# noahares/raxtax

Measured on AMD Instinct MI355X. Metric: classified queries/sec (whole node), higher is better.
Workload: dtype u32 bit-planes + f64

## Files before the change

### raxtax_amd/csrc/rtx_api_batch.hip

```cpp
#include "rtx_index.hpp"

#ifndef RTX_B2_HEAVY_PER_ATILE
#define RTX_B2_HEAVY_PER_ATILE 4u
#endif

namespace rtxi {

int bind(rtx_index *ix) {
    if (!ix) { set_error("null index handle"); return RTX_ERR_INVALID; }
    RTX_HIP(hipSetDevice(ix->device));
    return RTX_OK;
}

int ensure_events(rtx_index *ix, size_t count) {
    while (ix->events.size() < count) {
        hipEvent_t e;
        RTX_HIP(hipEventCreate(&e));
        ix->events.push_back(e);
    }
    return RTX_OK;
}


SubBatch sub_batch_of(rtx_index *ix, uint32_t sb, bool timed) {
// ... 524 lines not shown
        RTX_HIP(hipMemcpyAsync(&r.h_fin_sub[b.sb], r.d_fin_cursor.p, 8, hipMemcpyDeviceToHost, s));
    return RTX_OK;
}

static WalkParams walk_params(rtx_index *ix, const SubBatch &b, const double *prefix) {
    rtx_index::ResultSet &r = ix->res();
    WalkParams wp{};
    wp.status = r.d_status.p;
    wp.q0 = b.q0;
    wp.prefix = prefix;
    wp.n_bnd = ix->n_bnd;
    wp.rec = ix->d_noderec.p;
    wp.arena = r.d_arena.p;
    const bool side = b.cls->side;
    wp.arena_cap = side ? r.arena_cap : r.side_base;
    wp.arena_cursor = r.d_cursor.p + (side ? 1 : 0);
    wp.sub_alloc = !side && b.nq >= kWalkSubMinQueries && r.arena_cap < (1ull << 32) ? ix->d_sub_alloc.p : nullptr;
    wp.n_rows = r.d_n_rows.p;
    wp.row_start = r.d_row_start.p;
    wp.flags_out = r.d_flags.p;
    return wp;
}
static int reset_sub_alloc(rtx_index *ix, hipStream_t s) {
    if (ix->d_sub_alloc.p) RTX_HIP(hipMemsetAsync(ix->d_sub_alloc.p, 0, (size_t)kWalkSubAllocs * kWalkSubStride * 8, s));
    return RTX_OK;
}

int enqueue_walk(rtx_index *ix, const SubBatch &b, const double *prefix, hipStream_t s) {
    const WalkParams wp = walk_params(ix, b, prefix);
    int rc_r = wp.sub_alloc ? reset_sub_alloc(ix, s) : RTX_OK;
    if (rc_r) return rc_r;
    if (b.timed_all) RTX_HIP(hipEventRecord(stage_event(ix, b, RTX_STAGE_LINEAGE_WALK, 0), s));
    launch_lineage_walk(s, wp, b.nq);
    if (b.timed_all) RTX_HIP(hipEventRecord(stage_event(ix, b, RTX_STAGE_LINEAGE_WALK, 1), s));
    return RTX_OK;
}

int order_batch(rtx_index *ix, bool cluster) {
    const uint32_t n = (uint32_t)ix->n_q;
    rtx_index::ResultSet &r = ix->res();
    int rc;
    if ((rc = r.d_perm.alloc(n)) || (rc = r.d_iperm.alloc(n))) return rc;
    const bool multi = ix->n_cls > 1;
    const bool sketch = cluster && n > 2;
    if (sketch || multi) {
        if ((rc = ix->d_skey_in.alloc(n)) || (rc = ix->d_skey_out.alloc(n)) || (rc = ix->d_sidx.alloc(n))) return rc;
        size_t tmp = 0;
        if (cluster_sort(ix->stream, nullptr, &tmp, ix->d_skey_in.p, ix->d_skey_out.p, ix->d_sidx.p, r.d_perm.p, n, multi)) {
            set_error("radix sort: size query failed");
            return RTX_ERR_HIP;
        }
        if (ix->d_sort_tmp.n < tmp && (rc = ix->d_sort_tmp.alloc(tmp + 256))) return rc;
        if (sketch) {
            launch_sketch(ix->stream, ix->d_bases.p, ix->in[ix->cur_in].d_base_off.p, n, ix->d_skey_in.p, ix->d_sidx.p);
            if (ix->d_loc_table.p && ix->locator_opt)
                launch_locator(ix->stream, ix->d_bases.p, ix->in[ix->cur_in].d_base_off.p, n, ix->d_loc_table.p, ix->n_total, ix->d_skey_in.p);
        }
        if (multi) launch_class_keys(ix->stream, ix->d_skey_in.p, ix->in[ix->cur_in].d_base_off.p, n, ix->key_lim, !sketch, ix->d_sidx.p);
        tmp = ix->d_sort_tmp.n;
        if (cluster_sort(ix->stream, ix->d_sort_tmp.p, &tmp, ix->d_skey_in.p, ix->d_skey_out.p, ix->d_sidx.p, r.d_perm.p, n, multi)) {
            set_error("radix sort of the query sketches failed");
            return RTX_ERR_HIP;
        }
        launch_invert_perm(ix->stream, r.d_perm.p, n, r.d_iperm.p);
    } else {
        launch_identity_perm(ix->stream, n, r.d_perm.p, r.d_iperm.p);
    }
    RTX_HIP(hipGetLastError());
    return RTX_OK;
}

void record_batch(rtx_index *ix) {
    rtx_index::ResultSet &r = ix->res();
    r.n_q = ix->n_q;
    r.n_user = ix->strand_used ? ix->n_user : ix->n_q;
    r.has_peak = false;
    r.has_nearest = false;
    r.has_identity = false;
    r.profiled = false;
    r.n_sub = ix->n_sub_total();
    r.n_side = 0;
    for (uint32_t c = 0; c < ix->n_cls; c++)
        if (ix->cls[c].side) r.n_side += ix->cls[c].n_sub;
    r.in_set = ix->cur_in;
    r.dev_exact = ix->dev_exact_used;
    r.stream_dl = false;
}

int begin_run(rtx_index *ix, uint32_t *n_sub_out, bool *timed_out, bool cluster) {
    int rc_p = plan_sub_batches(ix);
    if (rc_p) return rc_p;
    const uint32_t n_sub = ix->n_sub_total();
    record_batch(ix);
    rtx_index::ResultSet &r = ix->res();
    const bool timed = n_sub <= 4096;
    if (timed) {
        int rc = ensure_events(ix, (size_t)n_sub * RTX_NUM_STAGES * 2);
        if (rc) return rc;
    }
    const bool ev_all = timed && ix->stage_timing;
    if (ev_all) RTX_HIP(hipEventRecord(ix->events[(size_t)RTX_STAGE_ORDER * 2], ix->stream));
    int rc_o = order_batch(ix, cluster);
    if (rc_o) return rc_o;
    if (ev_all) RTX_HIP(hipEventRecord(ix->events[(size_t)RTX_STAGE_ORDER * 2 + 1], ix->stream));
    {
        uint64_t n_side_q = 0;
        for (uint32_t c = 0; c < ix->n_cls; c++)
            if (ix->cls[c].side) n_side_q += ix->cls[c].n;
        const uint64_t side_rows = n_side_q ? n_side_q * kWalkMaxRows + 64 : 0;
// ... 696 lines not shown
```

### raxtax_amd/csrc/rtx_cluster.hip

```cpp
#include <cstring>

#include <hip/hip_runtime.h>
#include <rocprim/device/device_radix_sort.hpp>

#include "rtx_kernels.hpp"
#include "rtx_wave.hpp"

namespace rtx {

static constexpr int kSketchK = 12;
static constexpr uint32_t kSketchBits = 21;

__global__ __launch_bounds__(64) void sketch_kernel(const uint8_t *__restrict__ bases, const uint64_t *__restrict__ off,
                                                    uint64_t *__restrict__ keys, uint32_t *__restrict__ idx) {
    const uint32_t q = blockIdx.x, lane = threadIdx.x;
    const uint64_t b0 = off[q], len = off[q + 1] - b0;
    const uint8_t *seq = bases + b0;
    const uint32_t none = (1u << kSketchBits) - 1u;
    uint32_t m1 = none, m2 = none, m3 = none;
    if (len >= (uint64_t)kSketchK) {
        const uint64_t nwin = len - kSketchK + 1;
        const uint64_t wpl = (nwin + 63) / 64;
        const uint64_t w0 = (uint64_t)lane * wpl;
        const uint64_t w1 = w0 + wpl < nwin ? w0 + wpl : nwin;
        for (uint64_t i = w0; i < w1; i += 16) {
            unsigned long long v[4];
            __builtin_memcpy(v, seq + i, 32);
            const uint32_t nw = w1 - i < 16 ? (uint32_t)(w1 - i) : 16u;
            uint32_t code = 0, run = 0;
#pragma unroll
            for (int b = 0; b < 16 + kSketchK - 1; b++) {
                const uint32_t c = (uint32_t)(v[b >> 3] >> ((b & 7) * 8)) & 0xFFu;
                const bool ok = c == 1u || c == 2u || c == 4u || c == 8u;
                code = ((code << 2) | (((uint32_t)__ffs((int)c) - 1u) & 3u)) & 0xFFFFFFu;
                run = ok ? run + 1u : 0u;
                if (b >= kSketchK - 1 && (uint32_t)(b - (kSketchK - 1)) < nw && run >= (uint32_t)kSketchK) {
                    const uint64_t x = code;
                    const uint32_t h1 = (uint32_t)((x * 0x9E3779B97F4A7C15ull) >> (64 - kSketchBits));
                    const uint32_t h2 = (uint32_t)((x * 0xC2B2AE3D27D4EB4Full) >> (64 - kSketchBits));
                    const uint32_t h3 = (uint32_t)((x * 0x165667B19E3779F9ull) >> (64 - kSketchBits));
                    m1 = h1 < m1 ? h1 : m1;
                    m2 = h2 < m2 ? h2 : m2;
                    m3 = h3 < m3 ? h3 : m3;
                }
            }
        }
    }
#pragma unroll
    for (int d = 32; d >= 1; d >>= 1) {
        const uint32_t o1 = __shfl_xor(m1, d, 64), o2 = __shfl_xor(m2, d, 64), o3 = __shfl_xor(m3, d, 64);
        m1 = o1 < m1 ? o1 : m1;
        m2 = o2 < m2 ? o2 : m2;
        m3 = o3 < m3 ? o3 : m3;
    }
    if (lane == 0) {
        keys[q] = ((uint64_t)m1 << (2 * kSketchBits)) | ((uint64_t)m2 << kSketchBits) | m3;
        idx[q] = q;
    }
}

static constexpr uint32_t kLocNone = 0xFFFFFFFFu;
static constexpr uint32_t kLocMaxCount = 512;

__device__ __forceinline__ bool base_code(uint32_t c, uint32_t &two) {
    two = ((uint32_t)__ffs((int)c) - 1u) & 3u;
    return c == 1u || c == 2u || c == 4u || c == 8u;
}

__global__ __launch_bounds__(64) void loc_mark_kernel(const uint8_t *__restrict__ bases, const uint64_t *__restrict__ off,
                                                      uint64_t n_refs, uint32_t *__restrict__ pos_min, uint32_t *__restrict__ cnt) {
    const uint32_t lane = threadIdx.x;
    for (uint64_t r = blockIdx.x; r < n_refs; r += gridDim.x) {
        const uint64_t b0 = off[r], len = off[r + 1] - b0;
        if (len < (uint64_t)kSketchK) continue;
        const uint8_t *seq = bases + b0;
        const uint64_t nwin = len - kSketchK + 1;
        for (uint64_t w = lane; w < nwin; w += 64) {
            uint32_t code = 0;
            bool ok = true;
#pragma unroll
            for (int j = 0; j < kSketchK; j++) {
                uint32_t two;
                ok = base_code(seq[w + j], two) && ok;
                code = (code << 2) | two;
            }
            if (ok) {
                atomicMin(&pos_min[code], (uint32_t)r);
                atomicAdd(&cnt[code], 1u);
            }
        }
    }
}

__global__ __launch_bounds__(256) void loc_finish_kernel(uint32_t *__restrict__ pos_min, const uint32_t *__restrict__ cnt) {
    const uint32_t i = blockIdx.x * 256 + threadIdx.x;
    const uint32_t c = cnt[i];
    if (c == 0u || c > kLocMaxCount) pos_min[i] = kLocNone;
}

static constexpr uint32_t kLocMaxBins = 8192;
static constexpr uint32_t kLocFineDiv = 16;
static constexpr uint32_t kLocWin = 1024;
#ifndef RTX_LOC_STRIDE
#define RTX_LOC_STRIDE 2
#endif
static constexpr uint32_t kLocStride = RTX_LOC_STRIDE;

__device__ __forceinline__ void vote_bins(uint32_t *h, uint32_t b, bool valid, uint32_t lane) {
    unsigned long long pending = __ballot(valid);
#pragma unroll
    for (int r = 0; r < 2; r++) {
        if (!pending) return;
        const int first = __builtin_ctzll(pending);
        const uint32_t lead = (uint32_t)__builtin_amdgcn_readlane((int)b, first);
        const unsigned long long same = __ballot(valid && b == lead) & pending;
        if ((int)lane == first) atomicAdd(&h[lead >> 1], (uint32_t)__popcll(same) << ((lead & 1u) * 16u));
        pending &= ~same;
    }
    if ((pending >> lane) & 1ull) atomicAdd(&h[b >> 1], 1u << ((b & 1u) * 16u));
}

__global__ __launch_bounds__(64) void locator_kernel(const uint8_t *__restrict__ bases, const uint64_t *__restrict__ off,
                                                     const uint32_t *__restrict__ table, uint32_t bin_shift, uint32_t n_bins,
                                                     uint64_t *__restrict__ keys) {
    extern __shared__ __attribute__((aligned(16))) uint32_t h[];
    __shared__ uint32_t lcode[kLocWin / kLocStride];
    __shared__ uint32_t hf[kLocFineDiv + 2];
    const uint32_t q = blockIdx.x, lane = threadIdx.x;
    const uint64_t b0 = off[q], len = off[q + 1] - b0;
    if (len < (uint64_t)kSketchK) return;
    const uint64_t old_key = keys[q];
    const uint8_t *seq = bases + b0;
    const uint32_t nwin = (uint32_t)(len - kSketchK + 1 < (uint64_t)kLocWin ? len - kSketchK + 1 : kLocWin);
    const uint32_t words = n_bins / 2 + 2;
    for (uint32_t i = lane; i < (words + 3u) / 4u; i += 64) reinterpret_cast<uint4 *>(h)[i] = make_uint4(0u, 0u, 0u, 0u);
    if (lane < kLocFineDiv + 2) hf[lane] = 0;
    {
        const uint32_t wpl = (nwin + 63u) / 64u;
        const uint32_t w0 = lane * wpl, w1 = w0 + wpl < nwin ? w0 + wpl : nwin;
        static_assert(kLocWin <= 1024u && kLocWin % kLocStride == 0u, "a lane's run of windows fits one piece of 16");
        if (w0 < w1) {
            unsigned long long v[4];
            __builtin_memcpy(v, seq + w0, 32);
            const uint32_t nw = w1 - w0;
            uint32_t code = 0, run = 0;
#pragma unroll
            for (int b = 0; b < 16 + kSketchK - 1; b++) {
                uint32_t two;
                const bool ok = base_code((uint32_t)(v[b >> 3] >> ((b & 7) * 8)) & 0xFFu, two);
                code = ((code << 2) | two) & 0xFFFFFFu;
                run = ok ? run + 1u : 0u;
                if (b >= kSketchK - 1 && (uint32_t)(b - (kSketchK - 1)) < nw) {
                    const uint32_t w = w0 + (uint32_t)(b - (kSketchK - 1));
                    if (w % kLocStride == 0u) lcode[w / kLocStride] = run >= (uint32_t)kSketchK ? code : kLocNone;
                }
            }
        }
    }
    __builtin_amdgcn_fence(__ATOMIC_ACQ_REL, "wavefront");
    __builtin_amdgcn_wave_barrier();
    uint32_t any = 0;
    const uint32_t nlook = (nwin + kLocStride - 1u) / kLocStride;
    for (uint32_t j0 = 0; j0 < nlook; j0 += 256) {
        uint32_t pos[4];
#pragma unroll
        for (int u = 0; u < 4; u++) {
            const uint32_t j = j0 + (uint32_t)u * 64u + lane;
            const uint32_t code = j < nlook ? lcode[j] : kLocNone;
            pos[u] = table[code == kLocNone ? 0u : code];
            if (code == kLocNone) pos[u] = kLocNone;
        }
#pragma unroll
        for (int u = 0; u < 4; u++) {
            const uint32_t j = j0 + (uint32_t)u * 64u + lane;
            const bool valid = pos[u] != kLocNone;
            vote_bins(h, pos[u] >> bin_shift, valid, lane);
            if (j < nlook) lcode[j] = pos[u];
            any |= valid ? 1u : 0u;
        }
    }
    __builtin_amdgcn_fence(__ATOMIC_ACQ_REL, "wavefront");
    __builtin_amdgcn_wave_barrier();
    if (!__ballot(any != 0u)) return;
    auto bin = [&](uint32_t b) { return (h[b >> 1] >> ((b & 1u) * 16u)) & 0xFFFFu; };
    uint32_t best = 0;
    for (uint32_t k = lane; 2u * k < n_bins; k += 64) {
        const uint32_t w0 = h[k], w1 = h[k + 1u];
        const uint32_t v0 = (w0 & 0xFFFFu) + (w0 >> 16), v1 = (w0 >> 16) + (w1 & 0xFFFFu);
        const uint32_t c0 = (v0 << 16) | (0xFFFFu - 2u * k), c1 = 2u * k + 1u < n_bins ? (v1 << 16) | (0xFFFFu - (2u * k + 1u)) : 0u;
        best = c0 > best ? c0 : best;
        best = c1 > best ? c1 : best;
    }
    best = wave_max_u32(best);
    const uint32_t B = 0xFFFFu - (best & 0xFFFFu);
    const uint32_t lo = B << bin_shift;
    uint32_t fine = 0;
    if (bin_shift >= 4u) {
        const uint32_t fshift = bin_shift - 4u;
        for (uint32_t w0 = 0; w0 < nlook; w0 += 64) {
            const uint32_t w = w0 + lane;
            const uint32_t p = w < nlook ? lcode[w] : kLocNone;
            const bool in = p != kLocNone && p >= lo && ((p - lo) >> bin_shift) < 2u;
            vote_bins(hf, in ? (p - lo) >> fshift : 0u, in, lane);
        }
        __builtin_amdgcn_fence(__ATOMIC_ACQ_REL, "wavefront");
        __builtin_amdgcn_wave_barrier();
        uint32_t fb = 0;
        if (lane < 2u * kLocFineDiv) {
            const uint32_t v = ((hf[lane >> 1] >> ((lane & 1u) * 16u)) & 0xFFFFu) + ((hf[(lane + 1u) >> 1] >> (((lane + 1u) & 1u) * 16u)) & 0xFFFFu);
            fb = (v << 16) | (0xFFFFu - lane);
        }
        fb = wave_max_u32(fb);
        fine = 0xFFFFu - (fb & 0xFFFFu);
    }
    const uint64_t loc = ((uint64_t)B * kLocFineDiv + fine) & 0xFFFFFFull;
    if (lane == 0) keys[q] = (loc << 39) | (old_key >> 24);
}

__global__ __launch_bounds__(256) void class_keys_kernel(uint64_t *__restrict__ keys, const uint64_t *__restrict__ off, uint32_t n, uint64_t lim0,
                                                         uint64_t lim1, uint64_t lim2, uint64_t lim3, uint32_t shift, uint32_t from_index, uint32_t *__restrict__ idx) {
    const uint32_t q = blockIdx.x * 256 + threadIdx.x;
    if (q >= n) return;
    const uint64_t len = off[q + 1] - off[q];
    const uint64_t rank = (len > lim0 ? 1u : 0u) + (len > lim1 ? 1u : 0u) + (len > lim2 ? 1u : 0u) + (len > lim3 ? 1u : 0u);
    const uint64_t k = from_index ? (uint64_t)q : keys[q] >> shift;
    keys[q] = (rank << 61) | k;
    if (from_index) idx[q] = q;
}

__global__ __launch_bounds__(256) void invert_perm_kernel(const uint32_t *__restrict__ perm, uint32_t n, uint32_t *__restrict__ inv) {
    const uint32_t i = blockIdx.x * 256 + threadIdx.x;
    if (i < n) inv[perm[i]] = i;
}

__global__ __launch_bounds__(256) void identity_perm_kernel(uint32_t n, uint32_t *__restrict__ perm, uint32_t *__restrict__ inv) {
    const uint32_t i = blockIdx.x * 256 + threadIdx.x;
    if (i < n) { perm[i] = i; inv[i] = i; }
}

void launch_sketch(hipStream_t s, const uint8_t *bases, const uint64_t *off, uint32_t n_q, uint64_t *keys, uint32_t *idx) {
    hipLaunchKernelGGL(sketch_kernel, dim3(n_q), dim3(64), 0, s, bases, off, keys, idx);
}
void launch_loc_mark(hipStream_t s, const uint8_t *bases, const uint64_t *off, uint64_t n_refs, uint32_t *pos_min, uint32_t *cnt) {
    const uint32_t grid = (uint32_t)(n_refs < 65536u ? (n_refs ? n_refs : 1u) : 65536u);
    hipLaunchKernelGGL(loc_mark_kernel, dim3(grid), dim3(64), 0, s, bases, off, n_refs, pos_min, cnt);
}
void launch_loc_finish(hipStream_t s, uint32_t *pos_min, const uint32_t *cnt) {
    hipLaunchKernelGGL(loc_finish_kernel, dim3(kLocTableEntries / 256), dim3(256), 0, s, pos_min, cnt);
}
uint32_t loc_bin_shift(uint64_t n_refs) {
    uint32_t sh = 8;
    while (((n_refs + (1ull << sh) - 1) >> sh) + 1 > kLocMaxBins) sh++;
    return sh;
}
void launch_locator(hipStream_t s, const uint8_t *bases, const uint64_t *off, uint32_t n_q, const uint32_t *table, uint64_t n_refs,
                    uint64_t *keys) {
    const uint32_t sh = loc_bin_shift(n_refs);
    const uint32_t n_bins = (uint32_t)((n_refs + (1ull << sh) - 1) >> sh);
    hipLaunchKernelGGL(locator_kernel, dim3(n_q), dim3(64), ((n_bins / 2 + 2 + 3) & ~3u) * 4, s, bases, off, table, sh, n_bins, keys);
}
void launch_invert_perm(hipStream_t s, const uint32_t *perm, uint32_t n, uint32_t *inv) {
    hipLaunchKernelGGL(invert_perm_kernel, dim3((n + 255) / 256), dim3(256), 0, s, perm, n, inv);
}
void launch_identity_perm(hipStream_t s, uint32_t n, uint32_t *perm, uint32_t *inv) {
    hipLaunchKernelGGL(identity_perm_kernel, dim3((n + 255) / 256), dim3(256), 0, s, n, perm, inv);
}

void launch_class_keys(hipStream_t s, uint64_t *keys, const uint64_t *off, uint32_t n, const uint64_t lim[4], bool from_index, uint32_t *idx) {
    hipLaunchKernelGGL(class_keys_kernel, dim3((n + 255) / 256), dim3(256), 0, s, keys, off, n, lim[0], lim[1], lim[2], lim[3], 2u, from_index ? 1u : 0u, idx);
}

int cluster_sort(hipStream_t s, void *tmp, size_t *tmp_bytes, const uint64_t *keys_in, uint64_t *keys_out, const uint32_t *idx_in,
                 uint32_t *perm_out, size_t n, bool with_class) {
    const hipError_t e = rocprim::radix_sort_pairs(tmp, *tmp_bytes, keys_in, keys_out, idx_in, perm_out, n, 0, with_class ? 64u : 3 * kSketchBits, s);
    return e == hipSuccess ? 0 : 1;
}

}
```

### raxtax_amd/csrc/rtx_kernels.hip

```cpp
#include <hip/hip_runtime.h>

#include "rtx_kernels.hpp"
#include "rtx_math.hpp"
#include "rtx_wave.hpp"
#include "rtx_hit_common.hpp"
#include "rtx_walk.hpp"

namespace rtx {

static constexpr uint32_t kEmptyRow = 0xFFFFFFFFu;

__global__ __launch_bounds__(256) void bitmap_build_kernel(const uint64_t *__restrict__ off,
                                                           const uint32_t *__restrict__ post,
                                                           const uint32_t *__restrict__ row_of,
                                                           uint32_t *__restrict__ bitmap, uint32_t stride_words, uint32_t n_rows1,
                                                           uint32_t ref_lo, uint32_t ref_hi, uint32_t shift) {
    const uint32_t k = blockIdx.x;
    const uint32_t row = row_of[k];
    if (row == kEmptyRow) return;
    const uint64_t b = off[k], e = off[k + 1];
    for (uint64_t i = b + threadIdx.x; i < e; i += blockDim.x) {
        const uint32_t g = post[i];
        if (g < ref_lo || g >= ref_hi) continue;
        uint32_t word, bit;
// ... 32 lines not shown
    __syncthreads();
    for (uint32_t i = lane; i < 2048; i += 64)
        if (bm[i]) atomicOr(&present[i], bm[i]);
}

__global__ __launch_bounds__(64) void ref_bitmap_set_kernel(const uint8_t *__restrict__ bases,
                                                            const uint64_t *__restrict__ off, uint64_t n_refs,
                                                            const uint32_t *__restrict__ row_of,
                                                            uint32_t *__restrict__ bitmap, uint32_t stride_words, uint32_t n_rows1,
                                                            uint32_t shift) {
    const uint64_t r = blockIdx.x;
    if (r >= n_refs) return;
    const uint32_t lane = threadIdx.x;
    const uint64_t b0 = off[r], len = off[r + 1] - b0;
    uint32_t word, bitpos;
    ref_slot((uint32_t)(r >> shift), stride_words * 4u, word, bitpos);
    const uint32_t bit = 1u << bitpos;
    for (uint64_t w = lane; w + 8 <= len; w += 64) {
        uint32_t k;
        if (window_kmer(bases + b0, w, k)) atomicOr(&bitmap[bitmap_word(row_of[k], word, n_rows1)], bit);
    }
}

__global__ __launch_bounds__(256) void row_popcount_kernel(const uint32_t *__restrict__ row_of,
                                                           const uint32_t *__restrict__ bitmap, uint32_t stride_words, uint32_t n_rows1,
                                                           uint32_t *__restrict__ list_len) {
    __shared__ uint32_t part[4];
    const uint32_t k = blockIdx.x;
    const uint32_t row = row_of[k];
    if (row == kEmptyRow) {
        if (threadIdx.x == 0) list_len[k] = 0;
        return;
    }
    uint32_t c = 0;
    for (uint32_t i = threadIdx.x; i < stride_words; i += 256) c += __popc(bitmap[bitmap_word(row, i, n_rows1)]);
#pragma unroll
    for (int d = 32; d >= 1; d >>= 1) c += __shfl_xor(c, d, 64);
    if ((threadIdx.x & 63u) == 0) part[threadIdx.x >> 6] = c;
    __syncthreads();
    if (threadIdx.x == 0) list_len[k] = part[0] + part[1] + part[2] + part[3];
}

__device__ __forceinline__ unsigned long long transpose64(unsigned long long x, uint32_t lane) {
#pragma unroll
    for (int s = 32; s >= 1; s >>= 1) {
        const unsigned long long m = s == 32 ? 0x00000000FFFFFFFFull : s == 16 ? 0x0000FFFF0000FFFFull : s == 8 ? 0x00FF00FF00FF00FFull
                                   : s == 4 ? 0x0F0F0F0F0F0F0F0Full : s == 2 ? 0x3333333333333333ull : 0x5555555555555555ull;
        const unsigned long long y = __shfl_xor(x, s, 64);
        x = (lane & (uint32_t)s) ? (((y >> s) & m) | (x & ~m)) : ((x & m) | ((y & m) << s));
    }
    return x;
}

template <bool kTilesOnly>
__global__ __launch_bounds__(64) void kmer_extract_kernel(KmerParams p) {
    const uint32_t mode = kTilesOnly ? 2u : p.mode;
    __shared__ __attribute__((aligned(16))) uint32_t bm[kTilesOnly ? 64 : 2048];
    const uint32_t q = blockIdx.x;
    const uint32_t lane = threadIdx.x;
    const uint64_t gq = p.q0 + q;
    const uint64_t qin = p.perm[gq];
    const uint64_t b0 = p.base_off[qin];
    const uint64_t len = p.base_off[qin + 1] - b0;
    const uint8_t *seq = p.bases + b0;

    uint32_t t = 0, nrows = 0;
    unsigned long long hq = 0;
    uint32_t *rout = p.rows + (size_t)q * p.rstride;
    const unsigned long long lt_mask = (1ull << lane) - 1ull;
    if (mode == 2u) {
        nrows = p.nrows[q];
    } else {
    for (uint32_t i = lane; i < 2048; i += 64) bm[i] = 0;
    {
        uint32_t *h = p.hist + (size_t)q * p.hstride;
        for (uint32_t i = lane; i < p.hstride; i += 64) h[i] = 0;
    }
    if (q == 0u) {
#pragma unroll
        for (int k = 0; k < 3; k++)
            for (uint32_t i = lane; i < p.zero_n[k]; i += 64) p.zero[k][i] = 0;
    }
    __syncthreads();

    if (len >= 8) {
        const uint64_t nwin = len - 7;
        const uint64_t wpl = (nwin + 63) / 64;
        const uint64_t w0 = (uint64_t)lane * wpl;
        const uint64_t w1 = w0 + wpl < nwin ? w0 + wpl : nwin;
        for (uint64_t i = w0; i < w1; i += 16) {
            unsigned long long v[3];
            __builtin_memcpy(v, seq + i, 24);
            const uint32_t nw = w1 - i < 16 ? (uint32_t)(w1 - i) : 16u;
            uint32_t k = 0, run = 0;
#pragma unroll
            for (int b = 0; b < 23; b++) {
                const uint32_t c = (uint32_t)(v[b >> 3] >> ((b & 7) * 8)) & 0xFFu;
                const bool ok = c == 1u || c == 2u || c == 4u || c == 8u;
                k = ((k << 2) | (((uint32_t)__ffs((int)c) - 1u) & 3u)) & 0xFFFFu;
                run = ok ? run + 1u : 0u;
                if (b >= 7 && (uint32_t)(b - 7) < nw && run >= 8u) atomicOr(&bm[k >> 5], 1u << (k & 31u));
            }
        }
    }
    __syncthreads();

    uint16_t *kout = p.kmers + (size_t)q * p.kstride;
    const unsigned long long *bm64 = reinterpret_cast<const unsigned long long *>(bm);
    uint32_t base = 0;
    for (uint32_t r = 0; r < 16; r++) {
        unsigned long long word = bm64[r * 64 + lane];
        const uint32_t cnt = (uint32_t)__popcll(word);
        const uint32_t incl = wave_incl_scan_u32(cnt);
        uint32_t pos = base + incl - cnt;
        const uint32_t kbase = (r * 64 + lane) * 64;
        while (word) {
            const uint32_t bit = (uint32_t)__builtin_ctzll(word);
            word &= word - 1;
            if (pos < p.kstride) kout[pos] = (uint16_t)(kbase + bit);
            pos++;
        }
        base += (uint32_t)__builtin_amdgcn_readlane((int)incl, 63);
    }
    t = base;
    __syncthreads();
    const bool all_kmers = t > 65535u;

    const uint32_t tt = all_kmers ? 0u : (t < p.kstride ? t : p.kstride);
    for (uint32_t i0 = 0; i0 < tt; i0 += 256) {
        uint32_t kk[4], row[4], ll[4];
#pragma unroll
        for (int u = 0; u < 4; u++) {
            const uint32_t i = i0 + u * 64 + lane;
            kk[u] = i < tt ? (uint32_t)kout[i] : 0xFFFFFFFFu;
        }
#pragma unroll
        for (int u = 0; u < 4; u++) {
            row[u] = kEmptyRow;
            ll[u] = 0;
            if (kk[u] != 0xFFFFFFFFu) {
                const uint2 rl = p.row_len[kk[u]];
                row[u] = rl.x;
                ll[u] = rl.y;
            }
        }
#pragma unroll
        for (int u = 0; u < 4; u++) {
            hq += ll[u];
            const unsigned long long m = __ballot(row[u] != kEmptyRow);
            if (row[u] != kEmptyRow) rout[nrows + __popcll(m & lt_mask)] = row[u];
            nrows += (uint32_t)__popcll(m);
        }
    }
    for (uint32_t i = nrows + lane; i < ((nrows + 63u) & ~63u); i += 64) rout[i] = p.zero_row;
    __syncthreads();
    }
    if (mode == 1u) {
#pragma unroll
        for (int d = 32; d >= 1; d >>= 1) hq += __shfl_xor(hq, d, 64);
        if (lane == 0) { p.t[q] = t > 65535u ? 0u : t; p.nrows[q] = nrows; p.hq[gq] = hq; p.t_all[gq] = t; }
        return;
    }
    const uint32_t nchunks = (nrows + 63u) >> 6;
    const uint32_t *live = mode == 2u ? p.live + (size_t)q * p.live_words : nullptr;
    const uint32_t nt = p.ntiles;
    const uint32_t mstride = p.rstride >> 6;
    unsigned long long *dm = p.dmask + (size_t)q * nt * mstride;
    uint32_t *sout = p.srows + (size_t)q * nt * (kSegMaxSparseRows + 1);
    uint32_t nseg = 0;
    __shared__ unsigned long long l_sb[64];
    __shared__ uint32_t l_base[64];
    bool few_done = false;
    if (live && p.seg_blocks) {
        const uint32_t lw = (nt + 31u) >> 5;
        uint32_t nlive = 0;
        for (uint32_t w = 0; w < lw; w++) nlive += (uint32_t)__popc(live[w]);
        if (nlive <= kKmerFewLive) {
            for (uint32_t w = 0; w < lw; w++) {
                uint32_t bits = (uint32_t)__builtin_amdgcn_readfirstlane((int)live[w]);
                while (bits) {
                    const uint32_t tile = w * 32u + (uint32_t)__builtin_ctz(bits);
                    bits &= bits - 1u;
                    if (tile >= nt) break;
                    uint32_t cd = 0, cs = 0;
                    for (uint32_t c0 = 0; c0 < nchunks; c0 += 4) {
                        uint32_t row[4], cls[4];
#pragma unroll
                        for (int u = 0; u < 4; u++) {
                            const uint32_t i = (c0 + (uint32_t)u) * 64 + lane;
                            row[u] = i < nrows ? rout[i] : kEmptyRow;
                        }
#pragma unroll
                        for (int u = 0; u < 4; u++) {
                            const uint32_t r = row[u] == kEmptyRow ? 0u : row[u];
                            cls[u] = (p.segcls[(size_t)tile * p.cls_stride + (r >> 4)] >> ((r & 15u) * 2u)) & 3u;
                            if (row[u] == kEmptyRow) cls[u] = 0u;
                        }
                        uint32_t srank[4], slot[4];
                        bool take[4];
#pragma unroll
                        for (int u = 0; u < 4; u++) {
                            const uint32_t c = c0 + (uint32_t)u;
                            take[u] = false;
                            srank[u] = 0u;
                            if (c >= nchunks) continue;
// ... 829 lines not shown
```

### raxtax_amd/csrc/rtx_kernels.hpp

```cpp
#pragma once

#include <hip/hip_runtime.h>

#include <cstdint>

#include "raxtax_hip.h"
#include "rtx_math.hpp"

namespace rtx {

#ifndef RTX_NODE_TYPES_DEFINED
#define RTX_NODE_TYPES_DEFINED
enum NodeType : uint8_t { kInner = 0, kTaxon = 1, kSequence = 2 };
#endif

constexpr uint32_t kWalkMaxRows = 208;
constexpr uint32_t kSegPad = 8192;
__host__ __device__ inline uint32_t seg_pad(uint32_t i) { return kSegPad + ((i & 63u) << 2); }
constexpr uint32_t kKmerFewLive = 8;
constexpr uint32_t kHitListCap = 1024;

struct DevRow {
    uint32_t node;
    uint8_t k[RTX_MAX_DEPTH];
// ... 436 lines not shown
struct TailParams {
    RecordRef rec;
    const uint32_t *t;
    const double *table_z;
    uint32_t hstride;
    const uint8_t *bnd_bits;
    const uint32_t *bnd_rank;
    double *prefix;
    uint32_t *cnt_cursor;
    uint32_t cnt_cap;
    uint32_t *flags_out;
    uint32_t n_bnd;
    uint32_t nq;
    WalkParams walk;
    unsigned long long *prefix_stats;
    unsigned long long *stats;
};
void launch_records_tail(hipStream_t s, const TailParams &p, uint32_t nq);

void launch_bitmap_build(hipStream_t s, const uint64_t *off, const uint32_t *post, const uint32_t *row_of,
                         uint32_t *bitmap, uint32_t stride_words, uint32_t n_rows1, uint32_t ref_lo, uint32_t ref_hi, uint32_t shift = 0);
void launch_ref_kmer_mark(hipStream_t s, const uint8_t *bases, const uint64_t *off, uint64_t n_refs, uint32_t *present);
void launch_ref_bitmap_set(hipStream_t s, const uint8_t *bases, const uint64_t *off, uint64_t n_refs,
                           const uint32_t *row_of, uint32_t *bitmap, uint32_t stride_words, uint32_t n_rows1, uint32_t shift = 0);
void launch_row_len_pack(hipStream_t s, const uint32_t *row_of, const uint32_t *list_len, uint2 *out);
void launch_row_popcount(hipStream_t s, const uint32_t *row_of, const uint32_t *bitmap, uint32_t stride_words, uint32_t n_rows1,
                         uint32_t *list_len);
void launch_kmer_extract(hipStream_t s, const KmerParams &p, uint32_t nq);
void launch_hit_count(hipStream_t s, const HitParams &p, uint32_t nq, uint32_t ntiles, int planes);
void launch_pair_union(hipStream_t s, const uint32_t *rows, const uint32_t *nrows, uint32_t rstride, uint32_t nq, uint2 *urec,
                       uint32_t *nu, uint32_t ustride);
void launch_hit_count_pair(hipStream_t s, const HitParams &p, uint32_t nq, uint32_t ntiles, int planes);
void launch_live_items(hipStream_t s, const uint32_t *live, uint32_t live_words, uint32_t nq, uint32_t ntiles, uint32_t *items, uint32_t *n_items,
                       unsigned long long *stats);
void launch_hit_count_pair_bounds(hipStream_t s, const HitParams &p, uint32_t nq, uint32_t u_ntiles, int planes);
void launch_hit_count_pair_bounds_items(hipStream_t s, const HitParams &p, uint32_t nq, uint32_t u_ntiles, int planes);
void launch_fine_bounds(hipStream_t s, const HitParams &p, uint32_t nq, uint32_t f_ntiles, const uint32_t *pair_live, uint32_t *cnt,
                        uint32_t *items, uint32_t *n_items, int planes);
size_t prob_table_lds_bytes(uint32_t tmax);
void launch_prob_table(hipStream_t s, const ProbParams &p, uint32_t nq);
size_t prob_lookup_lds_bytes(uint32_t tmax);
void launch_prob_tables_build(hipStream_t s, const ProbTables &tb, const double *lf, const double *inv);
void launch_prob_order(hipStream_t s, const uint32_t *t, uint32_t nq, uint32_t *order);
void launch_prob_lookup(hipStream_t s, const ProbParams &p, const ProbTables &tb, uint32_t nq);
void launch_seg_popcount(hipStream_t s, const uint32_t *bitmap, uint32_t stride_bytes, uint32_t n_rows1, uint32_t ntiles, uint16_t *pop);
void launch_seg_emit(hipStream_t s, const uint32_t *bitmap, uint32_t stride_bytes, uint32_t n_rows1, uint32_t ntiles,
                     const uint32_t *seginfo, uint32_t seg_stride, uint16_t *slots);
void launch_sketch(hipStream_t s, const uint8_t *bases, const uint64_t *off, uint32_t n_q, uint64_t *keys, uint32_t *idx);
void launch_invert_perm(hipStream_t s, const uint32_t *perm, uint32_t n, uint32_t *inv);
constexpr uint32_t kLocTableEntries = 1u << 24;
void launch_loc_mark(hipStream_t s, const uint8_t *bases, const uint64_t *off, uint64_t n_refs, uint32_t *pos_min, uint32_t *cnt);
void launch_loc_finish(hipStream_t s, uint32_t *pos_min, const uint32_t *cnt);
void launch_locator(hipStream_t s, const uint8_t *bases, const uint64_t *off, uint32_t n_q, const uint32_t *table, uint64_t n_refs,
                    uint64_t *keys);
void launch_identity_perm(hipStream_t s, uint32_t n, uint32_t *perm, uint32_t *inv);
int cluster_sort(hipStream_t s, void *tmp, size_t *tmp_bytes, const uint64_t *keys_in, uint64_t *keys_out, const uint32_t *idx_in,
                 uint32_t *perm_out, size_t n, bool with_class = false);
void launch_class_keys(hipStream_t s, uint64_t *keys, const uint64_t *off, uint32_t n, const uint64_t lim[4], bool from_index, uint32_t *idx);
void launch_taxon_prefix(hipStream_t s, const PrefixParams &p, uint32_t nq);
void launch_lineage_walk(hipStream_t s, const WalkParams &p, uint32_t nq);
void launch_finalise(hipStream_t s, const FinaliseParams &p);
void launch_probs_expand(hipStream_t s, const uint16_t *counts, const double *tz, uint64_t n, double *out);
void launch_rehist(hipStream_t s, const uint16_t *counts, uint64_t npad, uint64_t n_refs, const uint32_t *t, uint32_t *hist,
                   uint32_t hstride, uint16_t *tile_max, uint32_t ntiles, uint32_t nq);
void launch_counts_unpack(hipStream_t s, const uint8_t *lo, const uint16_t *hi, uint64_t n, uint16_t *out);

}
```

### raxtax_amd/csrc/rtx_wave.hpp

```cpp
#pragma once

#include <hip/hip_runtime.h>

#include <cstdint>

namespace rtx {

__device__ __forceinline__ uint32_t lane_id() { return threadIdx.x & 63u; }

__device__ __forceinline__ uint32_t wave_incl_scan_u32(uint32_t v) {
    v += (uint32_t)__builtin_amdgcn_update_dpp(0, (int)v, 0x111, 0xF, 0xF, true);
    v += (uint32_t)__builtin_amdgcn_update_dpp(0, (int)v, 0x112, 0xF, 0xF, true);
    v += (uint32_t)__builtin_amdgcn_update_dpp(0, (int)v, 0x114, 0xF, 0xF, true);
    v += (uint32_t)__builtin_amdgcn_update_dpp(0, (int)v, 0x118, 0xF, 0xF, true);
    const uint32_t r0 = (uint32_t)__builtin_amdgcn_readlane((int)v, 15), r1 = (uint32_t)__builtin_amdgcn_readlane((int)v, 31),
                   r2 = (uint32_t)__builtin_amdgcn_readlane((int)v, 47);
    const uint32_t row = lane_id() >> 4;
    return v + (row == 0 ? 0u : (row == 1 ? r0 : (row == 2 ? r0 + r1 : r0 + r1 + r2)));
}

__device__ __forceinline__ uint32_t row16_max_u32(uint32_t v) {
    uint32_t o;
    o = (uint32_t)__builtin_amdgcn_update_dpp(0, (int)v, 0xB1, 0xF, 0xF, true); v = o > v ? o : v;
    o = (uint32_t)__builtin_amdgcn_update_dpp(0, (int)v, 0x4E, 0xF, 0xF, true); v = o > v ? o : v;
    o = (uint32_t)__builtin_amdgcn_update_dpp(0, (int)v, 0x141, 0xF, 0xF, true); v = o > v ? o : v;
    o = (uint32_t)__builtin_amdgcn_update_dpp(0, (int)v, 0x140, 0xF, 0xF, true); v = o > v ? o : v;
    return v;
}

__device__ __forceinline__ uint32_t row16_min_u32(uint32_t v) {
    uint32_t o;
    o = (uint32_t)__builtin_amdgcn_update_dpp(0, (int)v, 0xB1, 0xF, 0xF, true); v = o < v ? o : v;
    o = (uint32_t)__builtin_amdgcn_update_dpp(0, (int)v, 0x4E, 0xF, 0xF, true); v = o < v ? o : v;
    o = (uint32_t)__builtin_amdgcn_update_dpp(0, (int)v, 0x141, 0xF, 0xF, true); v = o < v ? o : v;
    o = (uint32_t)__builtin_amdgcn_update_dpp(0, (int)v, 0x140, 0xF, 0xF, true); v = o < v ? o : v;
    return v;
}

__device__ __forceinline__ uint32_t row16_sum_u32(uint32_t v) {
    v += (uint32_t)__builtin_amdgcn_update_dpp(0, (int)v, 0xB1, 0xF, 0xF, true);
    v += (uint32_t)__builtin_amdgcn_update_dpp(0, (int)v, 0x4E, 0xF, 0xF, true);
    v += (uint32_t)__builtin_amdgcn_update_dpp(0, (int)v, 0x141, 0xF, 0xF, true);
    v += (uint32_t)__builtin_amdgcn_update_dpp(0, (int)v, 0x140, 0xF, 0xF, true);
    return v;
}

__device__ __forceinline__ uint32_t wave_max_u32(uint32_t v) {
    v = row16_max_u32(v);
    const uint32_t a = (uint32_t)__builtin_amdgcn_readlane((int)v, 0), b = (uint32_t)__builtin_amdgcn_readlane((int)v, 16),
                   c = (uint32_t)__builtin_amdgcn_readlane((int)v, 32), d = (uint32_t)__builtin_amdgcn_readlane((int)v, 48);
    const uint32_t ab = a > b ? a : b, cd = c > d ? c : d;
    return ab > cd ? ab : cd;
}

__device__ __forceinline__ double wave_sum_f64(double v) {
#pragma unroll
    for (int d = 32; d >= 1; d >>= 1) v += __shfl_xor(v, d, 64);
    return v;
}

__device__ __forceinline__ double dpp_mov_f64(double v, int ctrl_sel) {
    int lo = __double2loint(v), hi = __double2hiint(v);
    switch (ctrl_sel) {
        case 0: lo = __builtin_amdgcn_update_dpp(0, lo, 0xB1, 0xF, 0xF, true); hi = __builtin_amdgcn_update_dpp(0, hi, 0xB1, 0xF, 0xF, true); break;
        case 1: lo = __builtin_amdgcn_update_dpp(0, lo, 0x4E, 0xF, 0xF, true); hi = __builtin_amdgcn_update_dpp(0, hi, 0x4E, 0xF, 0xF, true); break;
        case 2: lo = __builtin_amdgcn_update_dpp(0, lo, 0x141, 0xF, 0xF, true); hi = __builtin_amdgcn_update_dpp(0, hi, 0x141, 0xF, 0xF, true); break;
        case 3: lo = __builtin_amdgcn_update_dpp(0, lo, 0x140, 0xF, 0xF, true); hi = __builtin_amdgcn_update_dpp(0, hi, 0x140, 0xF, 0xF, true); break;
        default: lo = __builtin_amdgcn_update_dpp(0, lo, 0x128, 0xF, 0xF, true); hi = __builtin_amdgcn_update_dpp(0, hi, 0x128, 0xF, 0xF, true); break;
    }
    return __hiloint2double(hi, lo);
}
__device__ __forceinline__ double readlane_f64(double v, int l) {
    return __hiloint2double(__builtin_amdgcn_readlane(__double2hiint(v), l), __builtin_amdgcn_readlane(__double2loint(v), l));
}
__device__ __forceinline__ double wave_sum_f64_dpp(double v) {
    v += dpp_mov_f64(v, 0);
    v += dpp_mov_f64(v, 1);
    v += dpp_mov_f64(v, 2);
    v += dpp_mov_f64(v, 3);
    return (readlane_f64(v, 0) + readlane_f64(v, 16)) + (readlane_f64(v, 32) + readlane_f64(v, 48));
}

__device__ __forceinline__ double wave_sum8_f64(const double (&a)[8]) {
    const uint32_t lane = lane_id();
    const bool b2 = lane & 4u, b1 = lane & 2u, b0 = lane & 1u;
    double b[4], c[2];
#pragma unroll
    for (int j = 0; j < 4; j++) b[j] = (b2 ? a[j + 4] : a[j]) + dpp_mov_f64(b2 ? a[j] : a[j + 4], 2);
#pragma unroll
    for (int j = 0; j < 2; j++) c[j] = (b1 ? b[j + 2] : b[j]) + dpp_mov_f64(b1 ? b[j] : b[j + 2], 1);
    double d = (b0 ? c[1] : c[0]) + dpp_mov_f64(b0 ? c[0] : c[1], 0);
    d += dpp_mov_f64(d, 4);
    d += __shfl_xor(d, 16, 64);
    d += __shfl_xor(d, 32, 64);
    return d;
}

__device__ __forceinline__ double wave_prod_f64_dpp(double v) {
    v *= dpp_mov_f64(v, 0);
    v *= dpp_mov_f64(v, 1);
    v *= dpp_mov_f64(v, 2);
    v *= dpp_mov_f64(v, 3);
    return (readlane_f64(v, 0) * readlane_f64(v, 16)) * (readlane_f64(v, 32) * readlane_f64(v, 48));
}

// ... 33 lines not shown
```

Baseline: 13.30 million.

## Fuse minhash sketch into locator kernel and stage k-mer list in LDS

```diff
diff --git a/raxtax_amd/csrc/rtx_api_batch.hip b/raxtax_amd/csrc/rtx_api_batch.hip
--- a/raxtax_amd/csrc/rtx_api_batch.hip
+++ b/raxtax_amd/csrc/rtx_api_batch.hip
@@ -600,9 +600,10 @@
         }
         if (ix->d_sort_tmp.n < tmp && (rc = ix->d_sort_tmp.alloc(tmp + 256))) return rc;
         if (sketch) {
-            launch_sketch(ix->stream, ix->d_bases.p, ix->in[ix->cur_in].d_base_off.p, n, ix->d_skey_in.p, ix->d_sidx.p);
             if (ix->d_loc_table.p && ix->locator_opt)
-                launch_locator(ix->stream, ix->d_bases.p, ix->in[ix->cur_in].d_base_off.p, n, ix->d_loc_table.p, ix->n_total, ix->d_skey_in.p);
+                launch_locator(ix->stream, ix->d_bases.p, ix->in[ix->cur_in].d_base_off.p, n, ix->d_loc_table.p, ix->n_total, ix->d_skey_in.p, ix->d_sidx.p);
+            else
+                launch_sketch(ix->stream, ix->d_bases.p, ix->in[ix->cur_in].d_base_off.p, n, ix->d_skey_in.p, ix->d_sidx.p);
         }
         if (multi) launch_class_keys(ix->stream, ix->d_skey_in.p, ix->in[ix->cur_in].d_base_off.p, n, ix->key_lim, !sketch, ix->d_sidx.p);
         tmp = ix->d_sort_tmp.n;
diff --git a/raxtax_amd/csrc/rtx_cluster.hip b/raxtax_amd/csrc/rtx_cluster.hip
--- a/raxtax_amd/csrc/rtx_cluster.hip
+++ b/raxtax_amd/csrc/rtx_cluster.hip
@@ -10,51 +10,63 @@
 
 static constexpr int kSketchK = 12;
 static constexpr uint32_t kSketchBits = 21;
+
+template <class F>
+__device__ __forceinline__ void roll_windows16(const uint8_t *p, uint32_t nw, F f) {
+    unsigned long long v[4];
+    __builtin_memcpy(v, p, 32);
+    uint32_t code = 0, run = 0;
+#pragma unroll
+    for (int b = 0; b < 16 + kSketchK - 1; b++) {
+        const uint32_t c = (uint32_t)(v[b >> 3] >> ((b & 7) * 8)) & 0xFFu;
+        const bool ok = c == 1u || c == 2u || c == 4u || c == 8u;
+        code = ((code << 2) | (((uint32_t)__ffs((int)c) - 1u) & 3u)) & 0xFFFFFFu;
+        run = ok ? run + 1u : 0u;
+        if (b >= kSketchK - 1 && (uint32_t)(b - (kSketchK - 1)) < nw) f((uint32_t)(b - (kSketchK - 1)), code, run >= (uint32_t)kSketchK);
+    }
+}
+
+template <int kHashes>
+__device__ __forceinline__ void minhash_add(uint32_t code, uint32_t (&m)[kHashes]) {
+    constexpr uint64_t mult[3] = {0x9E3779B97F4A7C15ull, 0xC2B2AE3D27D4EB4Full, 0x165667B19E3779F9ull};
+    static_assert(kHashes >= 1 && kHashes <= 3, "three hashes are defined");
+#pragma unroll
+    for (int i = 0; i < kHashes; i++) {
+        const uint32_t h = (uint32_t)(((uint64_t)code * mult[i]) >> (64 - kSketchBits));
+        m[i] = h < m[i] ? h : m[i];
+    }
+}
+
+template <int kHashes>
+__device__ __forceinline__ void minhash_span(const uint8_t *seq, uint64_t lo, uint64_t hi, uint32_t lane, uint32_t (&m)[kHashes]) {
+    const uint64_t wpl = (hi - lo + 63) / 64;
+    const uint64_t w0 = lo + (uint64_t)lane * wpl;
+    const uint64_t w1 = w0 + wpl < hi ? w0 + wpl : hi;
+    for (uint64_t i = w0; i < w1; i += 16)
+        roll_windows16(seq + i, w1 - i < 16 ? (uint32_t)(w1 - i) : 16u, [&](uint32_t, uint32_t code, bool valid) {
+            if (valid) minhash_add(code, m);
+        });
+}
+
+static constexpr uint32_t kSketchNone = (1u << kSketchBits) - 1u;
+
+__device__ __forceinline__ uint64_t sketch_key(uint32_t m1, uint32_t m2, uint32_t m3) {
+    return ((uint64_t)m1 << (2 * kSketchBits)) | ((uint64_t)m2 << kSketchBits) | m3;
+}
+
+__device__ __forceinline__ uint64_t sketch_key_of(const uint8_t *seq, uint64_t len, uint32_t lane) {
+    uint32_t m[3] = {kSketchNone, kSketchNone, kSketchNone};
+    if (len >= (uint64_t)kSketchK) minhash_span(seq, 0, len - kSketchK + 1, lane, m);
+    return sketch_key(wave_min_u32(m[0]), wave_min_u32(m[1]), wave_min_u32(m[2]));
+}
 
 __global__ __launch_bounds__(64) void sketch_kernel(const uint8_t *__restrict__ bases, const uint64_t *__restrict__ off,
                                                     uint64_t *__restrict__ keys, uint32_t *__restrict__ idx) {
     const uint32_t q = blockIdx.x, lane = threadIdx.x;
     const uint64_t b0 = off[q], len = off[q + 1] - b0;
-    const uint8_t *seq = bases + b0;
-    const uint32_t none = (1u << kSketchBits) - 1u;
-    uint32_t m1 = none, m2 = none, m3 = none;
-    if (len >= (uint64_t)kSketchK) {
-        const uint64_t nwin = len - kSketchK + 1;
-        const uint64_t wpl = (nwin + 63) / 64;
-        const uint64_t w0 = (uint64_t)lane * wpl;
-        const uint64_t w1 = w0 + wpl < nwin ? w0 + wpl : nwin;
-        for (uint64_t i = w0; i < w1; i += 16) {
-            unsigned long long v[4];
-            __builtin_memcpy(v, seq + i, 32);
-            const uint32_t nw = w1 - i < 16 ? (uint32_t)(w1 - i) : 16u;
-            uint32_t code = 0, run = 0;
-#pragma unroll
-            for (int b = 0; b < 16 + kSketchK - 1; b++) {
-                const uint32_t c = (uint32_t)(v[b >> 3] >> ((b & 7) * 8)) & 0xFFu;
-                const bool ok = c == 1u || c == 2u || c == 4u || c == 8u;
-                code = ((code << 2) | (((uint32_t)__ffs((int)c) - 1u) & 3u)) & 0xFFFFFFu;
-                run = ok ? run + 1u : 0u;
-                if (b >= kSketchK - 1 && (uint32_t)(b - (kSketchK - 1)) < nw && run >= (uint32_t)kSketchK) {
-                    const uint64_t x = code;
-                    const uint32_t h1 = (uint32_t)((x * 0x9E3779B97F4A7C15ull) >> (64 - kSketchBits));
-                    const uint32_t h2 = (uint32_t)((x * 0xC2B2AE3D27D4EB4Full) >> (64 - kSketchBits));
-                    const uint32_t h3 = (uint32_t)((x * 0x165667B19E3779F9ull) >> (64 - kSketchBits));
-                    m1 = h1 < m1 ? h1 : m1;
-                    m2 = h2 < m2 ? h2 : m2;
-                    m3 = h3 < m3 ? h3 : m3;
-                }
-            }
-        }
-    }
-#pragma unroll
-    for (int d = 32; d >= 1; d >>= 1) {
-        const uint32_t o1 = __shfl_xor(m1, d, 64), o2 = __shfl_xor(m2, d, 64), o3 = __shfl_xor(m3, d, 64);
-        m1 = o1 < m1 ? o1 : m1;
-        m2 = o2 < m2 ? o2 : m2;
-        m3 = o3 < m3 ? o3 : m3;
-    }
+    const uint64_t key = sketch_key_of(bases + b0, len, lane);
     if (lane == 0) {
-        keys[q] = ((uint64_t)m1 << (2 * kSketchBits)) | ((uint64_t)m2 << kSketchBits) | m3;
+        keys[q] = key;
         idx[q] = q;
     }
 }
@@ -122,15 +134,19 @@
 
 __global__ __launch_bounds__(64) void locator_kernel(const uint8_t *__restrict__ bases, const uint64_t *__restrict__ off,
                                                      const uint32_t *__restrict__ table, uint32_t bin_shift, uint32_t n_bins,
-                                                     uint64_t *__restrict__ keys) {
+                                                     uint64_t *__restrict__ keys, uint32_t *__restrict__ idx) {
     extern __shared__ __attribute__((aligned(16))) uint32_t h[];
     __shared__ uint32_t lcode[kLocWin / kLocStride];
     __shared__ uint32_t hf[kLocFineDiv + 2];
     const uint32_t q = blockIdx.x, lane = threadIdx.x;
     const uint64_t b0 = off[q], len = off[q + 1] - b0;
-    if (len < (uint64_t)kSketchK) return;
-    const uint64_t old_key = keys[q];
+    if (lane == 0) idx[q] = q;
     const uint8_t *seq = bases + b0;
+    if (len < (uint64_t)kSketchK) {
+        if (lane == 0) keys[q] = sketch_key(kSketchNone, kSketchNone, kSketchNone);
+        return;
+    }
+    uint32_t m[2] = {kSketchNone, kSketchNone};
     const uint32_t nwin = (uint32_t)(len - kSketchK + 1 < (uint64_t)kLocWin ? len - kSketchK + 1 : kLocWin);
     const uint32_t words = n_bins / 2 + 2;
     for (uint32_t i = lane; i < (words + 3u) / 4u; i += 64) reinterpret_cast<uint4 *>(h)[i] = make_uint4(0u, 0u, 0u, 0u);
@@ -139,23 +155,14 @@
         const uint32_t wpl = (nwin + 63u) / 64u;
         const uint32_t w0 = lane * wpl, w1 = w0 + wpl < nwin ? w0 + wpl : nwin;
         static_assert(kLocWin <= 1024u && kLocWin % kLocStride == 0u, "a lane's run of windows fits one piece of 16");
-        if (w0 < w1) {
-            unsigned long long v[4];
-            __builtin_memcpy(v, seq + w0, 32);
-            const uint32_t nw = w1 - w0;
-            uint32_t code = 0, run = 0;
-#pragma unroll
-            for (int b = 0; b < 16 + kSketchK - 1; b++) {
-                uint32_t two;
-                const bool ok = base_code((uint32_t)(v[b >> 3] >> ((b & 7) * 8)) & 0xFFu, two);
-                code = ((code << 2) | two) & 0xFFFFFFu;
-                run = ok ? run + 1u : 0u;
-                if (b >= kSketchK - 1 && (uint32_t)(b - (kSketchK - 1)) < nw) {
-                    const uint32_t w = w0 + (uint32_t)(b - (kSketchK - 1));
-                    if (w % kLocStride == 0u) lcode[w / kLocStride] = run >= (uint32_t)kSketchK ? code : kLocNone;
-                }
-            }
-        }
+        if (w0 < w1)
+            roll_windows16(seq + w0, w1 - w0, [&](uint32_t j, uint32_t code, bool valid) {
+                const uint32_t w = w0 + j;
+                if (w % kLocStride == 0u) lcode[w / kLocStride] = valid ? code : kLocNone;
+                if (valid) minhash_add(code, m);
+            });
+        const uint64_t total = len - kSketchK + 1;
+        if (total > (uint64_t)kLocWin) minhash_span(seq, kLocWin, total, lane, m);
     }
     __builtin_amdgcn_fence(__ATOMIC_ACQ_REL, "wavefront");
     __builtin_amdgcn_wave_barrier();
@@ -181,7 +188,11 @@
     }
     __builtin_amdgcn_fence(__ATOMIC_ACQ_REL, "wavefront");
     __builtin_amdgcn_wave_barrier();
-    if (!__ballot(any != 0u)) return;
+    if (!__ballot(any != 0u)) {
+        const uint64_t key = sketch_key_of(seq, len, lane);
+        if (lane == 0) keys[q] = key;
+        return;
+    }
     auto bin = [&](uint32_t b) { return (h[b >> 1] >> ((b & 1u) * 16u)) & 0xFFFFu; };
     uint32_t best = 0;
     for (uint32_t k = lane; 2u * k < n_bins; k += 64) {
@@ -214,7 +225,8 @@
         fine = 0xFFFFu - (fb & 0xFFFFu);
     }
     const uint64_t loc = ((uint64_t)B * kLocFineDiv + fine) & 0xFFFFFFull;
-    if (lane == 0) keys[q] = (loc << 39) | (old_key >> 24);
+    const uint32_t m1 = wave_min_u32(m[0]), m2 = wave_min_u32(m[1]);
+    if (lane == 0) keys[q] = (loc << 39) | (sketch_key(m1, m2, 0u) >> 24);
 }
 
 __global__ __launch_bounds__(256) void class_keys_kernel(uint64_t *__restrict__ keys, const uint64_t *__restrict__ off, uint32_t n, uint64_t lim0,
@@ -254,10 +266,10 @@
     return sh;
 }
 void launch_locator(hipStream_t s, const uint8_t *bases, const uint64_t *off, uint32_t n_q, const uint32_t *table, uint64_t n_refs,
-                    uint64_t *keys) {
+                    uint64_t *keys, uint32_t *idx) {
     const uint32_t sh = loc_bin_shift(n_refs);
     const uint32_t n_bins = (uint32_t)((n_refs + (1ull << sh) - 1) >> sh);
-    hipLaunchKernelGGL(locator_kernel, dim3(n_q), dim3(64), ((n_bins / 2 + 2 + 3) & ~3u) * 4, s, bases, off, table, sh, n_bins, keys);
+    hipLaunchKernelGGL(locator_kernel, dim3(n_q), dim3(64), ((n_bins / 2 + 2 + 3) & ~3u) * 4, s, bases, off, table, sh, n_bins, keys, idx);
 }
 void launch_invert_perm(hipStream_t s, const uint32_t *perm, uint32_t n, uint32_t *inv) {
     hipLaunchKernelGGL(invert_perm_kernel, dim3((n + 255) / 256), dim3(256), 0, s, perm, n, inv);
diff --git a/raxtax_amd/csrc/rtx_kernels.hip b/raxtax_amd/csrc/rtx_kernels.hip
--- a/raxtax_amd/csrc/rtx_kernels.hip
+++ b/raxtax_amd/csrc/rtx_kernels.hip
@@ -108,6 +108,9 @@
     return x;
 }
 
+__device__ __forceinline__ uint32_t kmer_set_slot(uint32_t k) { return k ^ ((k >> 5) & 0x3C0u); }
+static constexpr uint32_t kKmerStage = 4096;
+
 template <bool kTilesOnly>
 __global__ __launch_bounds__(64) void kmer_extract_kernel(KmerParams p) {
     const uint32_t mode = kTilesOnly ? 2u : p.mode;
@@ -155,40 +158,56 @@
                 const bool ok = c == 1u || c == 2u || c == 4u || c == 8u;
                 k = ((k << 2) | (((uint32_t)__ffs((int)c) - 1u) & 3u)) & 0xFFFFu;
                 run = ok ? run + 1u : 0u;
-                if (b >= 7 && (uint32_t)(b - 7) < nw && run >= 8u) atomicOr(&bm[k >> 5], 1u << (k & 31u));
+                if (b >= 7 && (uint32_t)(b - 7) < nw && run >= 8u) {
+                    const uint32_t ks = kmer_set_slot(k);
+                    atomicOr(&bm[ks >> 5], 1u << (ks & 31u));
+                }
             }
         }
     }
     __syncthreads();
 
     uint16_t *kout = p.kmers + (size_t)q * p.kstride;
-    const unsigned long long *bm64 = reinterpret_cast<const unsigned long long *>(bm);
-    uint32_t base = 0;
-    for (uint32_t r = 0; r < 16; r++) {
-        unsigned long long word = bm64[r * 64 + lane];
-        const uint32_t cnt = (uint32_t)__popcll(word);
+    uint16_t *stage = reinterpret_cast<uint16_t *>(bm);
+    {
+        const unsigned long long *bm64 = reinterpret_cast<const unsigned long long *>(bm);
+        const uint32_t sw = (lane >> 1) & 15u;
+        unsigned long long w[16];
+        uint32_t cnt = 0;
+#pragma unroll
+        for (int j = 0; j < 16; j++) {
+            w[j] = bm64[lane * 16u + ((uint32_t)j ^ sw)];
+            cnt += (uint32_t)__popcll(w[j]);
+        }
         const uint32_t incl = wave_incl_scan_u32(cnt);
-        uint32_t pos = base + incl - cnt;
-        const uint32_t kbase = (r * 64 + lane) * 64;
-        while (word) {
-            const uint32_t bit = (uint32_t)__builtin_ctzll(word);
-            word &= word - 1;
-            if (pos < p.kstride) kout[pos] = (uint16_t)(kbase + bit);
-            pos++;
-        }
-        base += (uint32_t)__builtin_amdgcn_readlane((int)incl, 63);
-    }
-    t = base;
+        t = (uint32_t)__builtin_amdgcn_readlane((int)incl, 63);
+        uint32_t pos = incl - cnt;
+        __syncthreads();
+#pragma unroll
+        for (int j = 0; j < 16; j++) {
+            unsigned long long word = w[j];
+            const uint32_t kbase = (lane * 16u + (uint32_t)j) * 64u;
+            while (word) {
+                const uint32_t bit = (uint32_t)__builtin_ctzll(word);
+                word &= word - 1;
+                if (pos < kKmerStage) stage[pos] = (uint16_t)(kbase + bit);
+                else if (pos < p.kstride) kout[pos] = (uint16_t)(kbase + bit);
+                pos++;
+            }
+        }
+    }
     __syncthreads();
     const bool all_kmers = t > 65535u;
 
     const uint32_t tt = all_kmers ? 0u : (t < p.kstride ? t : p.kstride);
     for (uint32_t i0 = 0; i0 < tt; i0 += 256) {
         uint32_t kk[4], row[4], ll[4];
+        const bool staged = i0 < kKmerStage;
 #pragma unroll
         for (int u = 0; u < 4; u++) {
             const uint32_t i = i0 + u * 64 + lane;
-            kk[u] = i < tt ? (uint32_t)kout[i] : 0xFFFFFFFFu;
+            kk[u] = 0xFFFFFFFFu;
+            if (i < tt) kk[u] = staged ? (uint32_t)stage[i] : (uint32_t)kout[i];
         }
 #pragma unroll
         for (int u = 0; u < 4; u++) {
@@ -207,6 +226,10 @@
             if (row[u] != kEmptyRow) rout[nrows + __popcll(m & lt_mask)] = row[u];
             nrows += (uint32_t)__popcll(m);
         }
+    }
+    {
+        const uint32_t ns = t < p.kstride ? (t < kKmerStage ? t : kKmerStage) : (p.kstride < kKmerStage ? p.kstride : kKmerStage);
+        for (uint32_t i = lane; i < ns; i += 64) kout[i] = stage[i];
     }
     for (uint32_t i = nrows + lane; i < ((nrows + 63u) & ~63u); i += 64) rout[i] = p.zero_row;
     __syncthreads();
diff --git a/raxtax_amd/csrc/rtx_kernels.hpp b/raxtax_amd/csrc/rtx_kernels.hpp
--- a/raxtax_amd/csrc/rtx_kernels.hpp
+++ b/raxtax_amd/csrc/rtx_kernels.hpp
@@ -512,7 +512,7 @@
 void launch_loc_mark(hipStream_t s, const uint8_t *bases, const uint64_t *off, uint64_t n_refs, uint32_t *pos_min, uint32_t *cnt);
 void launch_loc_finish(hipStream_t s, uint32_t *pos_min, const uint32_t *cnt);
 void launch_locator(hipStream_t s, const uint8_t *bases, const uint64_t *off, uint32_t n_q, const uint32_t *table, uint64_t n_refs,
-                    uint64_t *keys);
+                    uint64_t *keys, uint32_t *idx);
 void launch_identity_perm(hipStream_t s, uint32_t n, uint32_t *perm, uint32_t *inv);
 int cluster_sort(hipStream_t s, void *tmp, size_t *tmp_bytes, const uint64_t *keys_in, uint64_t *keys_out, const uint32_t *idx_in,
                  uint32_t *perm_out, size_t n, bool with_class = false);
diff --git a/raxtax_amd/csrc/rtx_wave.hpp b/raxtax_amd/csrc/rtx_wave.hpp
--- a/raxtax_amd/csrc/rtx_wave.hpp
+++ b/raxtax_amd/csrc/rtx_wave.hpp
@@ -51,6 +51,14 @@
                    c = (uint32_t)__builtin_amdgcn_readlane((int)v, 32), d = (uint32_t)__builtin_amdgcn_readlane((int)v, 48);
     const uint32_t ab = a > b ? a : b, cd = c > d ? c : d;
     return ab > cd ? ab : cd;
+}
+
+__device__ __forceinline__ uint32_t wave_min_u32(uint32_t v) {
+    v = row16_min_u32(v);
+    const uint32_t a = (uint32_t)__builtin_amdgcn_readlane((int)v, 0), b = (uint32_t)__builtin_amdgcn_readlane((int)v, 16),
+                   c = (uint32_t)__builtin_amdgcn_readlane((int)v, 32), d = (uint32_t)__builtin_amdgcn_readlane((int)v, 48);
+    const uint32_t ab = a < b ? a : b, cd = c < d ? c : d;
+    return ab < cd ? ab : cd;
 }
 
 __device__ __forceinline__ double wave_sum_f64(double v) {
```

Result: faster. 13.62 million (median of 6 runs) (+2.4%).
